# DIAGNijmegen/bodyct-dram-emph-subtype

Measured on AMD Instinct MI355X. Metric: CT volumes/sec (train step, 1x128x256x256), higher is better.
Workload: dtype f32; 1 GPU; BASELINE configs[1]: resnet18segcls train step (fwd+loss+bwd+Adam), batch 2/GPU, 1x128x256x256, fp32, inputs resident in HBM; global_batch=2, parallelism=dp1, hip_graph=False, streams=2

## Files before the change

bodyct-dram-emph-subtype_amd/csrc/conv_wino2d.hip:

```cpp
#include <stdlib.h>
#include "common.h"

namespace {

constexpr int W2_TZ16 = 16;
constexpr int W2_BK = 16;

struct W2dGeom {
  int B, D, H, W;
  int Ci, No;
  int nz, ny, nx, tiles_per_b, n_tiles, nblk;
};

__device__ __attribute__((aligned(16))) float g_w2d_zero[4];

__device__ constexpr int kBP[4][2] = {{0, 2}, {1, 2}, {1, 2}, {1, 3}};
__device__ constexpr float kBS[4][2] = {{1.f, -1.f}, {1.f, 1.f}, {-1.f, 1.f}, {1.f, -1.f}};
__device__ constexpr float kAT[2][4] = {{1.f, 1.f, 1.f, 0.f}, {0.f, 1.f, -1.f, -1.f}};

__device__ __forceinline__ int bswz(int n) {
  const int v = (n >> 2) & 7;
  return (v & 3) ^ ((v >> 2) * 3);
}

template <bool NEG>
__device__ __forceinline__ void pk_acc(f32x16& y, const f32x16& t) {
  typedef float f32x2 __attribute__((ext_vector_type(2)));
#pragma unroll
  for (int i = 0; i < 8; ++i) {
    f32x2 yy = {y[2 * i], y[2 * i + 1]};
    const f32x2 tt = {t[2 * i], t[2 * i + 1]};
    if (NEG) asm volatile("v_pk_add_f32 %0, %0, %1 neg_lo:[0,1] neg_hi:[0,1]" : "+v"(yy) : "v"(tt));
    else asm volatile("v_pk_add_f32 %0, %0, %1" : "+v"(yy) : "v"(tt));
    y[2 * i] = yy[0];
    y[2 * i + 1] = yy[1];
  }
}
template <int NJ>
__device__ __forceinline__ void mfma_result_wait(f32x16 (&t)[NJ]) {
  if (NJ == 2) asm volatile("s_nop 15\n\ts_nop 3" : "+v"(t[0]), "+v"(t[NJ - 1]));
  else asm volatile("s_nop 15\n\ts_nop 3" : "+v"(t[0]));
}

__device__ __forceinline__ int kx(int off, int gk) {
  if (gk == 0) return off;
  int r;
  asm volatile("v_xor_b32 %0, 8, %1" : "=v"(r) : "v"(off));
  return r;
}

template <int NJ, int NW = 8, int WS = 2>
__global__ __launch_bounds__(64 * NW, NW == 4 ? 2 : 1) void conv_wino2d_kernel(const float* __restrict__ in, const float* __restrict__ u2,
                                                              const float* __restrict__ bias, float* __restrict__ out,
                                                              float* __restrict__ stats, const float* __restrict__ add,
                                                              const float* __restrict__ gate, const W2dGeom g) {
  constexpr int W2_TZ = 2 * NW;
  constexpr int W2_HROWS = (W2_TZ + 2) * 10 * 10;
  constexpr int W2_NPIECE = (W2_HROWS + 15) / 16;
  constexpr int W2_HQ = (W2_NPIECE + NW - 1) / NW;
  constexpr int W2_HALO = W2_NPIECE * 256;
  constexpr int BN = 32 * NJ;
  constexpr int BROWS = 3 * BN;
  constexpr int BST = BROWS * 16;
  constexpr int BPIECE = BROWS / 16;
  constexpr int PB = (BPIECE + NW - 1) / NW;
  static_assert(WS != 3 || (NW == 4 && NJ == 2), "tap ring: one DMA piece per wave and tap");
  constexpr int TAP = BN * 16;
  __shared__ __attribute__((aligned(1024))) float lds[W2_HALO];
  __shared__ __attribute__((aligned(1024))) float wsa0[TAP], wsa1[TAP], wsa2[TAP];
  __shared__ __attribute__((aligned(1024))) float wsb0[WS == 2 ? TAP : 64], wsb1[WS == 2 ? TAP : 64],
      wsb2[WS == 2 ? TAP : 64];
  __shared__ int htab[W2_NPIECE * 16];
  float* halo = lds;

  const int tid = threadIdx.x;
  const int lane = tid & 63;
  const int wave = __builtin_amdgcn_readfirstlane(tid >> 6);

  int L = xcd_remap(blockIdx.x, g.nblk);
  const int n_tile = L % g.n_tiles;
  const int mt = L / g.n_tiles;
  const int b = mt / g.tiles_per_b;
  int r = mt - b * g.tiles_per_b;
  const int txi = r % g.nx; r /= g.nx;
  const int tyi = r % g.ny;
  const int tzi = r / g.ny;
  const int n0 = n_tile * BN;
  const int z0 = tzi * W2_TZ, y0 = tyi * 8, x0 = txi * 8;

  const int pslot = lane & 3;
  for (int rp = tid; rp < W2_NPIECE * 16; rp += 64 * NW) {
    const int yh = (rp / 10) % 10;
    const int rl = rp ^ ((yh >> 1) & 1);
    const int zh = rl / 100, xh = rl % 10;
    const int zi = z0 + zh - 1, yi = y0 + yh - 1, xi = x0 + xh - 1;
    const bool v = (rp < W2_HROWS) & (zi >= 0) & (zi < g.D) & (yi >= 0) & (yi < g.H) & (xi >= 0) & (xi < g.W);
    htab[rp] = v ? ((((b * g.D + zi) * g.H + yi) * g.W + xi) * g.Ci) | ((xh >> 2) & 1) | (((yh >> 2) & 1) << 1) : -1;
  }
  int boff[PB];
#pragma unroll
  for (int j = 0; j < PB; ++j) {
    int row = 16 * (wave + NW * j) + (lane >> 2);
    if (row >= BROWS) row = 0;
    const int a = row / BN, n = row - a * BN;
    boff[j] = (a * g.No + n0 + n) * g.Ci + (pslot ^ bswz(n)) * 4;
  }
  const long xi_stride = 3L * g.No * g.Ci;

  auto issue_halo = [&](int c) __attribute__((always_inline)) {
#pragma unroll 1
    for (int q = 0; q < W2_HQ; ++q) {
      if (wave + NW * q < W2_NPIECE) {
        const int ho = htab[16 * (wave + NW * q) + (lane >> 2)];
        const float* src = ho >= 0 ? in + (long)((ho & ~3) + ((pslot ^ (ho & 3)) << 2) + c * W2_BK) : g_w2d_zero;
        __builtin_amdgcn_global_load_lds((const __attribute__((address_space(1))) void*)src,
                                         (__attribute__((address_space(3))) void*)(halo + (wave + NW * q) * 256), 16, 0,
                                         0);
      }
    }
  };
  auto issue_b = [&](int c, int xi, int stage, int only = -1) __attribute__((always_inline)) {
#pragma unroll
    for (int j = 0; j < PB; ++j) {
      if ((only < 0 || only == j) && wave + NW * j < BPIECE) {
        const float* src = u2 + xi * xi_stride + c * W2_BK + boff[j];
        const int pb = wave + NW * j, tap = pb / (BN / 16), pin = pb - tap * (BN / 16);
        float* slot = stage == 0 ? (tap == 0 ? wsa0 : (tap == 1 ? wsa1 : wsa2)) : (tap == 0 ? wsb0 : (tap == 1 ? wsb1 : wsb2));
        __builtin_amdgcn_global_load_lds((const __attribute__((address_space(1))) void*)src,
                                         (__attribute__((address_space(3))) void*)(slot + pin * 256), 16, 0, 0);
      }
    }
  };

  f32x16 yacc[2][2][NJ];
#pragma unroll
  for (int oy = 0; oy < 2; ++oy)
#pragma unroll
    for (int ox = 0; ox < 2; ++ox)
#pragma unroll
      for (int nj = 0; nj < NJ; ++nj)
#pragma unroll
        for (int e = 0; e < 16; ++e) yacc[oy][ox][nj][e] = 0.f;

  const int li = lane & 31, lh = lane >> 5;
  const int zl = li >> 4, ty = (li >> 2) & 3, tx = li & 3;
  int abase[4][4];
#pragma unroll
  for (int p = 0; p < 4; ++p)
#pragma unroll
    for (int q = 0; q < 4; ++q) {
      const int yh = 2 * ty + p, xh = 2 * tx + q;
      const int rl = ((2 * wave + zl) * 10 + yh) * 10 + xh;
      abase[p][q] = (rl ^ ((yh >> 1) & 1)) * 16 + ((lh ^ (((xh >> 2) & 1) | (((yh >> 2) & 1) << 1))) * 4);
    }
  const int bbase = li * 16 + ((lh ^ bswz(li)) * 4);
  const int nchunk = g.Ci / W2_BK;

  for (int c = 0; c < nchunk; ++c) {
    __syncthreads();
    issue_halo(c);
    issue_b(c, 0, 0);
#pragma unroll
    for (int xi = 0; xi < 16; ++xi) {
      if (WS != 3 || xi == 0) __syncthreads();
      const int stage = WS == 2 ? (xi & 1) : 0;
      if (WS == 2 && xi + 1 < 16) issue_b(c, xi + 1, stage ^ 1);
      const int xy = xi >> 2, xx = xi & 3;
      const int p0 = kBP[xy][0], p1 = kBP[xy][1], q0 = kBP[xx][0], q1 = kBP[xx][1];
      const float s00 = kBS[xy][0] * kBS[xx][0], s01 = kBS[xy][0] * kBS[xx][1];
      const float s10 = kBS[xy][1] * kBS[xx][0], s11 = kBS[xy][1] * kBS[xx][1];
      f32x16 t[NJ];
#pragma unroll
      for (int a = 0; a < 3; ++a) {
        const float* wtap = stage == 0 ? (a == 0 ? wsa0 : (a == 1 ? wsa1 : wsa2)) : (a == 0 ? wsb0 : (a == 1 ? wsb1 : wsb2));
#pragma unroll
        for (int gk = 0; gk < 2; ++gk) {
          const f32x4 r00 = *reinterpret_cast<const f32x4*>(halo + kx(abase[p0][q0], gk) + a * 1600);
          const f32x4 r01 = *reinterpret_cast<const f32x4*>(halo + kx(abase[p0][q1], gk) + a * 1600);
          const f32x4 r10 = *reinterpret_cast<const f32x4*>(halo + kx(abase[p1][q0], gk) + a * 1600);
          const f32x4 r11 = *reinterpret_cast<const f32x4*>(halo + kx(abase[p1][q1], gk) + a * 1600);
          const f32x4 av = (s00 * r00 + s01 * r01) + (s10 * r10 + s11 * r11);
          f32x4 bf[NJ];
#pragma unroll
          for (int nj = 0; nj < NJ; ++nj)
            bf[nj] = *reinterpret_cast<const f32x4*>(wtap + nj * 32 * 16 + kx(bbase, gk));
#pragma unroll
          for (int e = 0; e < 4; ++e) {
#pragma unroll
            for (int nj = 0; nj < NJ; ++nj) {
              if (a == 0 && gk == 0 && e == 0) {
                f32x16 zero;
#pragma unroll
                for (int i = 0; i < 16; ++i) zero[i] = 0.f;
                t[nj] = __builtin_amdgcn_mfma_f32_32x32x2f32(av[e], bf[nj][e], zero, 0, 0, 0);
              } else {
                t[nj] = __builtin_amdgcn_mfma_f32_32x32x2f32(av[e], bf[nj][e], t[nj], 0, 0, 0);
              }
            }
          }
          __builtin_amdgcn_sched_barrier(0);
        }
        if (WS == 3 && !(xi == 15 && a == 2)) {
          if (xi == 15 && a >= 1) asm volatile("s_waitcnt vmcnt(0)");
          else asm volatile("s_waitcnt vmcnt(1)");
          __builtin_amdgcn_s_barrier();
          if (xi + 1 < 16) issue_b(c, xi + 1, 0, a);
        }
      }
      mfma_result_wait<NJ>(t);
#pragma unroll
      for (int oy = 0; oy < 2; ++oy)
#pragma unroll
        for (int ox = 0; ox < 2; ++ox) {
          const float cf = kAT[oy][xy] * kAT[ox][xx];
          if (cf != 0.f) {
#pragma unroll
            for (int nj = 0; nj < NJ; ++nj) {
              if (cf > 0.f) pk_acc<false>(yacc[oy][ox][nj], t[nj]);
              else pk_acc<true>(yacc[oy][ox][nj], t[nj]);
            }
          }
        }
      __builtin_amdgcn_sched_barrier(0);
      if (WS == 1 && xi + 1 < 16) {
        __syncthreads();
        issue_b(c, xi + 1, 0);
      }
    }
  }

  int lhe = lh, lie = li;
  asm volatile("" : "+v"(lhe), "+v"(lie));
  constexpr int P = 32 * NJ + 8;
  constexpr int Q = 8 * NJ;
  constexpr int VPP = 64 / Q;
  static_assert(NW * 32 * P <= W2_HALO, "turn regions fit the halo buffer");
  __syncthreads();
  float* reg = lds + wave * (32 * P);
  const int cq = lane % Q, rs = lane / Q;
  f32x4 s1 = {0.f, 0.f, 0.f, 0.f}, s2 = {0.f, 0.f, 0.f, 0.f}, bv = {0.f, 0.f, 0.f, 0.f};
  if (bias) bv = *reinterpret_cast<const f32x4*>(bias + n0 + 4 * cq);
#pragma unroll
  for (int oy = 0; oy < 2; ++oy)
#pragma unroll
    for (int ox = 0; ox < 2; ++ox) {
#pragma unroll
      for (int e = 0; e < 16; ++e)
#pragma unroll
        for (int nj = 0; nj < NJ; ++nj)
          reg[((e & 3) + 8 * (e >> 2) + 4 * lhe) * P + nj * 32 + lie] = yacc[oy][ox][nj][e];
#pragma unroll
      for (int ps = 0; ps < 32 / VPP; ++ps) {
        const int row = ps * VPP + rs;
        const int zo = z0 + 2 * wave + (row >> 4);
        const int yo = y0 + 2 * ((row >> 2) & 3) + oy, xo = x0 + 2 * (row & 3) + ox;
        f32x4 v = *reinterpret_cast<const f32x4*>(reg + row * P + 4 * cq);
        if ((zo < g.D) & (yo < g.H) & (xo < g.W)) {
          const long o = ((((long)b * g.D + zo) * g.H + yo) * g.W + xo) * g.No + n0 + 4 * cq;
          v += bv;
          if (add) {
            const f32x4 av = *reinterpret_cast<const f32x4*>(add + o);
            if (gate) {
              const f32x4 gv = *reinterpret_cast<const f32x4*>(gate + o);
#pragma unroll
              for (int j = 0; j < 4; ++j) v[j] += gv[j] > 0.f ? av[j] : 0.f;
            } else {
              v += av;
            }
          }
          *reinterpret_cast<f32x4*>(out + o) = v;
          s1 += v;
          s2 += v * v;
        }
      }
    }
  if (stats) {
#pragma unroll
    for (int j = 0; j < 4; ++j)
#pragma unroll
      for (int o = Q; o < 64; o <<= 1) {
        s1[j] += __shfl_xor(s1[j], o, 64);
        s2[j] += __shfl_xor(s2[j], o, 64);
      }
    __syncthreads();
    float* red = lds;
    if (rs == 0) {
#pragma unroll
      for (int j = 0; j < 4; ++j) {
        red[(wave * 2 + 0) * BN + 4 * cq + j] = s1[j];
        red[(wave * 2 + 1) * BN + 4 * cq + j] = s2[j];
      }
    }
    __syncthreads();
    if (tid < 2 * BN) {
      const int which = tid / BN, cc = tid - which * BN;
      float v = 0.f;
#pragma unroll
      for (int w = 0; w < NW; ++w) v += red[(w * 2 + which) * BN + cc];
      stats[((long)mt * 2 + which) * g.No + n0 + cc] = v;
    }
  }
}

constexpr int V2_TZ = 8;
constexpr int V2_HROWS = 10 * 10 * 10;
constexpr int V2_NPIECE = (V2_HROWS + 15) / 16;
constexpr int V2_HALO = V2_NPIECE * 256;

template <bool NEG>
__device__ __forceinline__ void pk_acc4(f32x4& y, const f32x4& t) {
  typedef float f32x2 __attribute__((ext_vector_type(2)));
#pragma unroll
  for (int i = 0; i < 2; ++i) {
    f32x2 yy = {y[2 * i], y[2 * i + 1]};
    const f32x2 tt = {t[2 * i], t[2 * i + 1]};
    if (NEG) asm volatile("v_pk_add_f32 %0, %0, %1 neg_lo:[0,1] neg_hi:[0,1]" : "+v"(yy) : "v"(tt));
    else asm volatile("v_pk_add_f32 %0, %0, %1" : "+v"(yy) : "v"(tt));
    y[2 * i] = yy[0];
    y[2 * i + 1] = yy[1];
  }
}
template <int NB>
__device__ __forceinline__ void mfma16_result_wait(f32x4 (&t)[NB]) {
  if (NB == 4) asm volatile("s_nop 12" : "+v"(t[0]), "+v"(t[1]), "+v"(t[2]), "+v"(t[NB - 1]));
  else asm volatile("s_nop 12" : "+v"(t[0]), "+v"(t[NB - 1]));
}

__device__ __forceinline__ int bswz16(int n) { return (0x78 >> (2 * ((n >> 2) & 3))) & 3; }

template <int NB>
__global__ __launch_bounds__(512) void conv_wino2d16_kernel(const float* __restrict__ in, const float* __restrict__ u2,
                                                            const float* __restrict__ bias, float* __restrict__ out,
                                                            float* __restrict__ stats, const float* __restrict__ add,
                                                            const float* __restrict__ gate, const W2dGeom g) {
  constexpr int BN = 16 * NB;
  constexpr int BROWS = 3 * BN;
  constexpr int BST = BROWS * 16;
  constexpr int BPIECE = BROWS / 16;
  constexpr int PB = (BPIECE + 7) / 8;
  __shared__ __attribute__((aligned(1024))) float lds[V2_HALO];
  __shared__ __attribute__((aligned(1024))) float halo1[V2_HALO];
  __shared__ __attribute__((aligned(1024))) float wst0[BST], wst1[BST];
  __shared__ int htab[V2_NPIECE * 16];

  const int tid = threadIdx.x;
  const int lane = tid & 63;
  const int wave = __builtin_amdgcn_readfirstlane(tid >> 6);

  int L = xcd_remap(blockIdx.x, g.nblk);
  const int n_tile = L % g.n_tiles;
  const int mt = L / g.n_tiles;
  const int b = mt / g.tiles_per_b;
  int r = mt - b * g.tiles_per_b;
  const int txi = r % g.nx; r /= g.nx;
  const int tyi = r % g.ny;
  const int tzi = r / g.ny;
  const int n0 = n_tile * BN;
  const int z0 = tzi * V2_TZ, y0 = tyi * 8, x0 = txi * 8;

  const int pslot = lane & 3;
  for (int rp = tid; rp < V2_NPIECE * 16; rp += 512) {
    const int yh = (rp / 10) % 10;
    const int rl = rp ^ ((yh >> 1) & 1);
    const int zh = rl / 100, xh = rl % 10;
    const int zi = z0 + zh - 1, yi = y0 + yh - 1, xi = x0 + xh - 1;
    const bool v = (rp < V2_HROWS) & (zi >= 0) & (zi < g.D) & (yi >= 0) & (yi < g.H) & (xi >= 0) & (xi < g.W);
    htab[rp] = v ? ((((b * g.D + zi) * g.H + yi) * g.W + xi) * g.Ci) | ((xh >> 2) & 1) | (((yh >> 2) & 1) << 1) : -1;
  }
  int boff[PB];
#pragma unroll
  for (int j = 0; j < PB; ++j) {
    int row = 16 * (wave + 8 * j) + (lane >> 2);
    if (row >= BROWS) row = 0;
    const int a = row / BN, n = row - a * BN;
    boff[j] = (a * g.No + n0 + n) * g.Ci + (pslot ^ bswz16(n)) * 4;
  }
  const long xi_stride = 3L * g.No * g.Ci;

  auto issue_halo_piece = [&](int c, int p, float* buf) __attribute__((always_inline)) {
    const int ho = htab[16 * p + (lane >> 2)];
    const float* src = ho >= 0 ? in + (long)((ho & ~3) + ((pslot ^ (ho & 3)) << 2) + c * W2_BK) : g_w2d_zero;
    __builtin_amdgcn_global_load_lds((const __attribute__((address_space(1))) void*)src,
                                     (__attribute__((address_space(3))) void*)(buf + p * 256), 16, 0, 0);
  };
  auto issue_b = [&](int c, int xi, int stage) __attribute__((always_inline)) {
#pragma unroll
    for (int j = 0; j < PB; ++j) {
      if (wave + 8 * j < BPIECE) {
        const float* src = u2 + xi * xi_stride + c * W2_BK + boff[j];
        __builtin_amdgcn_global_load_lds((const __attribute__((address_space(1))) void*)src,
                                         (__attribute__((address_space(3))) void*)((stage ? wst1 : wst0) + (wave + 8 * j) * 256),
                                         16, 0, 0);
      }
    }
  };

  f32x4 yacc[2][2][NB];
#pragma unroll
  for (int oy = 0; oy < 2; ++oy)
#pragma unroll
    for (int ox = 0; ox < 2; ++ox)
#pragma unroll
      for (int cb = 0; cb < NB; ++cb)
#pragma unroll
        for (int e = 0; e < 4; ++e) yacc[oy][ox][cb][e] = 0.f;

  const int lr = lane & 15, kq = lane >> 4;
  const int ty = lr >> 2, tx = lr & 3;
  int abase[4][4];
#pragma unroll
  for (int p = 0; p < 4; ++p)
#pragma unroll
    for (int q = 0; q < 4; ++q) {
      const int yh = 2 * ty + p, xh = 2 * tx + q;
      const int rl = (wave * 10 + yh) * 10 + xh;
      abase[p][q] = (rl ^ ((yh >> 1) & 1)) * 16 + ((kq ^ (((xh >> 2) & 1) | (((yh >> 2) & 1) << 1))) * 4);
    }
  const int bbase = lr * 16 + ((kq ^ bswz16(lr)) * 4);
  const int nchunk = g.Ci / W2_BK;

  __syncthreads();
#pragma unroll 1
  for (int q = 0; q < 8; ++q)
    if (wave + 8 * q < V2_NPIECE) issue_halo_piece(0, wave + 8 * q, lds);
  issue_b(0, 0, 0);

  auto chunk = [&](const int c, const float* hb, float* hn) __attribute__((always_inline)) {
#pragma unroll
    for (int xi = 0; xi < 16; ++xi) {
      __syncthreads();
      if (xi + 1 < 16) issue_b(c, xi + 1, (xi + 1) & 1);
      else if (c + 1 < nchunk) issue_b(c + 1, 0, 0);
      if (c + 1 < nchunk) {
        const int w4 = wave - 4 * (xi & 1);
        const int p = xi * 4 + w4;
        if (w4 >= 0 && w4 < 4 && p < V2_NPIECE) issue_halo_piece(c + 1, p, hn);
      }
      const int xy = xi >> 2, xx = xi & 3;
      const int p0 = kBP[xy][0], p1 = kBP[xy][1], q0 = kBP[xx][0], q1 = kBP[xx][1];
      const float s00 = kBS[xy][0] * kBS[xx][0], s01 = kBS[xy][0] * kBS[xx][1];
      const float s10 = kBS[xy][1] * kBS[xx][0], s11 = kBS[xy][1] * kBS[xx][1];
      const float* bs = (xi & 1) ? wst1 : wst0;
      f32x4 t[NB];
#pragma unroll
      for (int a = 0; a < 3; ++a) {
        const f32x4 r00 = *reinterpret_cast<const f32x4*>(hb + abase[p0][q0] + a * 1600);
        const f32x4 r01 = *reinterpret_cast<const f32x4*>(hb + abase[p0][q1] + a * 1600);
        const f32x4 r10 = *reinterpret_cast<const f32x4*>(hb + abase[p1][q0] + a * 1600);
        const f32x4 r11 = *reinterpret_cast<const f32x4*>(hb + abase[p1][q1] + a * 1600);
        f32x4 bf[NB];
#pragma unroll
        for (int cb = 0; cb < NB; ++cb)
          bf[cb] = *reinterpret_cast<const f32x4*>(bs + (a * BN + cb * 16) * 16 + bbase);
        const f32x4 av = (s00 * r00 + s01 * r01) + (s10 * r10 + s11 * r11);
#pragma unroll
        for (int e = 0; e < 4; ++e) {
#pragma unroll
          for (int cb = 0; cb < NB; ++cb) {
            if (a == 0 && e == 0) {
              const f32x4 zero = {0.f, 0.f, 0.f, 0.f};
              t[cb] = __builtin_amdgcn_mfma_f32_16x16x4f32(av[e], bf[cb][e], zero, 0, 0, 0);
            } else {
              t[cb] = __builtin_amdgcn_mfma_f32_16x16x4f32(av[e], bf[cb][e], t[cb], 0, 0, 0);
            }
          }
        }
      }
      mfma16_result_wait<NB>(t);
#pragma unroll
      for (int oy = 0; oy < 2; ++oy)
#pragma unroll
        for (int ox = 0; ox < 2; ++ox) {
          const float cf = kAT[oy][xy] * kAT[ox][xx];
          if (cf != 0.f) {
#pragma unroll
            for (int cb = 0; cb < NB; ++cb) {
              if (cf > 0.f) pk_acc4<false>(yacc[oy][ox][cb], t[cb]);
              else pk_acc4<true>(yacc[oy][ox][cb], t[cb]);
            }
          }
        }
    }
  };
  for (int c = 0; c < nchunk; c += 2) {
    chunk(c, lds, halo1);
    if (c + 1 < nchunk) chunk(c + 1, halo1, lds);
  }

  float s1[NB], s2[NB], bv[NB];
#pragma unroll
  for (int cb = 0; cb < NB; ++cb) {
    s1[cb] = 0.f;
    s2[cb] = 0.f;
    bv[cb] = bias ? bias[n0 + cb * 16 + lr] : 0.f;
  }
  const int zo = z0 + wave;
#pragma unroll
  for (int i = 0; i < 4; ++i) {
#pragma unroll
    for (int oy = 0; oy < 2; ++oy)
#pragma unroll
      for (int ox = 0; ox < 2; ++ox) {
        const int yo = y0 + 2 * kq + oy, xo = x0 + 2 * i + ox;
        if ((zo < g.D) & (yo < g.H) & (xo < g.W)) {
          const long o = ((((long)b * g.D + zo) * g.H + yo) * g.W + xo) * g.No + n0 + lr;
#pragma unroll
          for (int cb = 0; cb < NB; ++cb) {
            float v = yacc[oy][ox][cb][i] + bv[cb];
            if (add) {
              const float av = add[o + cb * 16];
              v += gate ? (gate[o + cb * 16] > 0.f ? av : 0.f) : av;
            }
            out[o + cb * 16] = v;
            s1[cb] += v;
            s2[cb] += v * v;
          }
        }
      }
  }
  if (stats) {
    __syncthreads();
    float* red = lds;
#pragma unroll
    for (int cb = 0; cb < NB; ++cb) {
      float t1 = s1[cb] + __shfl_xor(s1[cb], 16, 64);
      float t2 = s2[cb] + __shfl_xor(s2[cb], 16, 64);
      t1 += __shfl_xor(t1, 32, 64);
      t2 += __shfl_xor(t2, 32, 64);
      if (kq == 0) {
        red[(wave * 2 + 0) * BN + cb * 16 + lr] = t1;
        red[(wave * 2 + 1) * BN + cb * 16 + lr] = t2;
      }
    }
    __syncthreads();
    if (tid < 2 * BN) {
      const int which = tid / BN, cc = tid - which * BN;
      float v = 0.f;
#pragma unroll
      for (int w = 0; w < 8; ++w) v += red[(w * 2 + which) * BN + cc];
      stats[((long)mt * 2 + which) * g.No + n0 + cc] = v;
    }
  }
}

__device__ __forceinline__ void g4_2d(const float a0, const float a1, const float a2, float* r) {
  const float h = 0.5f * (a0 + a2);
  r[0] = a0;
  r[1] = h + 0.5f * a1;
  r[2] = h - 0.5f * a1;
  r[3] = a2;
}

__global__ __launch_bounds__(256) void wino2d_weight_kernel(const float* __restrict__ w, float* __restrict__ uf,
                                                            float* __restrict__ ub, const int Cout, const int Cin) {
  const bool bwd = blockIdx.y == 1;
  float* dst = bwd ? ub : uf;
  if (!dst) return;
  const long n = (long)Cout * Cin;
  const long i = blockIdx.x * 256L + threadIdx.x;
  if (i >= n) return;
  int co, ci;
  if (!bwd) { ci = (int)(i % Cin); co = (int)(i / Cin); }
  else { co = (int)(i % Cout); ci = (int)(i / Cout); }
  const float* src = w + ((long)co * Cin + ci) * 27;
  float gw[3][3][3];
#pragma unroll
  for (int t = 0; t < 27; ++t) (&gw[0][0][0])[t] = src[bwd ? 26 - t : t];
#pragma unroll
  for (int a = 0; a < 3; ++a) {
    float p[3][4], u[4][4];
#pragma unroll
    for (int ky = 0; ky < 3; ++ky) g4_2d(gw[a][ky][0], gw[a][ky][1], gw[a][ky][2], p[ky]);
#pragma unroll
    for (int x = 0; x < 4; ++x) {
      float col[4];
      g4_2d(p[0][x], p[1][x], p[2][x], col);
#pragma unroll
      for (int y = 0; y < 4; ++y) u[y][x] = col[y];
    }
#pragma unroll
    for (int xi = 0; xi < 16; ++xi) dst[((long)xi * 3 + a) * n + i] = u[xi >> 2][xi & 3];
  }
}

bool w2d_ok(const DramConvDesc* d, int K, int N) {
  if (!d) return false;
  if (d->B < 1 || d->D < 1 || d->H < 1 || d->W < 1) return false;
  if (d->k != 3 || d->stride != 1 || d->dil != 1 || d->pad != 1) return false;
  if (d->Do != d->D || d->Ho != d->H || d->Wo != d->W) return false;
  if (K < 16 || K % 16 != 0 || N < 32 || N % 32 != 0) return false;
  const long long cmax = K > N ? K : N;
  return (long long)d->B * d->D * d->H * d->W * cmax < (1LL << 31);
}

int w2d_variant(const DramConvDesc* d, int n_tiles, int BN) {
  if (const char* e = tune_env("DRAM_W2D_V")) {
    const int v = atoi(e);
    if (v >= 1 && v <= 3) return v;
  }
  const int z16 = (d->D + 15) / 16, z8 = (d->D + 7) / 8;
  const long cols = (long)d->B * ((d->H + 7) / 8) * ((d->W + 7) / 8) * n_tiles;
  if (BN == 64 && cols * z8 >= 1024) return 3;
  if (z16 * 16 != z8 * 8) return 2;
  auto fill = [](long wgs) { return (double)wgs / (double)(((wgs + 255) / 256) * 256); };
  return fill(cols * z16) + 0.05 < fill(cols * z8) ? 2 : 1;
}

W2dGeom make_w2d(const DramConvDesc* d, int K, int N, int BN, int* variant = nullptr) {
  W2dGeom g{};
  g.B = d->B; g.D = d->D; g.H = d->H; g.W = d->W; g.Ci = K; g.No = N;
  g.n_tiles = N / BN;
  const int v = w2d_variant(d, g.n_tiles, BN);
  if (variant) *variant = v;
  const int tz = v == 1 ? W2_TZ16 : V2_TZ;
  g.nz = (g.D + tz - 1) / tz;
  g.ny = (g.H + 7) / 8;
  g.nx = (g.W + 7) / 8;
  g.tiles_per_b = g.nz * g.ny * g.nx;
  g.nblk = g.B * g.tiles_per_b * g.n_tiles;
  return g;
}

int run_w2d(const float* in, const float* u2, const float* bias, const float* add, const float* gate, float* out,
            float* stats, const DramConvDesc* d, int K, int N, hipStream_t s) {
  const int BN = N % 64 == 0 ? 64 : 32;
  int variant = 1;
  const W2dGeom g = make_w2d(d, K, N, BN, &variant);
  const double vox_pad = (double)g.B * g.tiles_per_b * (variant == 1 ? W2_TZ16 : V2_TZ) * 64.0;
  const double vox = (double)g.B * g.D * g.H * g.W;
  DramProf prof(DRAM_FAM_CONV_WINO2D, variant * 100 + BN, 2.0 * vox_pad * K * N * 12.0,
                4.0 * (vox * (K + N * (1.0 + (add ? 1 : 0) + (gate ? 1 : 0))) + 48.0 * K * N), s,
                2.0 * vox * K * N * 27.0);
  if (variant == 1) {
    if (BN == 64)
      hipLaunchKernelGGL((conv_wino2d_kernel<2>), dim3(g.nblk), dim3(512), 0, s, in, u2, bias, out, stats, add, gate, g);
    else
      hipLaunchKernelGGL((conv_wino2d_kernel<1>), dim3(g.nblk), dim3(512), 0, s, in, u2, bias, out, stats, add, gate, g);
  } else if (variant == 3) {
    if (BN == 64)
      hipLaunchKernelGGL((conv_wino2d_kernel<2, 4, 3>), dim3(g.nblk), dim3(256), 0, s, in, u2, bias, out, stats, add, gate, g);
    else
      hipLaunchKernelGGL((conv_wino2d_kernel<1, 4, 1>), dim3(g.nblk), dim3(256), 0, s, in, u2, bias, out, stats, add, gate, g);
  } else {
    if (BN == 64)
      hipLaunchKernelGGL((conv_wino2d16_kernel<4>), dim3(g.nblk), dim3(512), 0, s, in, u2, bias, out, stats, add, gate, g);
    else
      hipLaunchKernelGGL((conv_wino2d16_kernel<2>), dim3(g.nblk), dim3(512), 0, s, in, u2, bias, out, stats, add, gate, g);
  }
  DRAM_LAUNCH_CHECK();
  return DRAM_OK;
}

}

extern "C" int dram_wino2d_applicable(const DramConvDesc* d) {
  return (d && w2d_ok(d, d->Cin, d->Cout) && w2d_ok(d, d->Cout, d->Cin)) ? 1 : 0;
}

extern "C" int dram_wino2d_num_stat_rows(const DramConvDesc* d) {
  if (!dram_wino2d_applicable(d)) return DRAM_ERR_UNSUPPORTED;
  const W2dGeom g = make_w2d(d, d->Cin, d->Cout, d->Cout % 64 == 0 ? 64 : 32);
  return g.B * g.tiles_per_b;
}

extern "C" int dram_wino2d_pack_weight(const float* w, float* uf, float* ub, int Cout, int Cin, dram_stream_t stream) {
  if (!w || (!uf && !ub) || Cout < 1 || Cin < 1) return DRAM_ERR_BAD_ARG;
  const long n = (long)Cout * Cin;
  DramProf prof(DRAM_FAM_WEIGHT_PACK, 2, 0.0, 4.0 * (double)n * (27.0 + (uf ? 48 : 0) + (ub ? 48 : 0)),
                (hipStream_t)stream);
  hipLaunchKernelGGL(wino2d_weight_kernel, dim3((unsigned)((n + 255) / 256), 2), dim3(256), 0, (hipStream_t)stream, w,
                     uf, ub, Cout, Cin);
  DRAM_LAUNCH_CHECK();
  return DRAM_OK;
}

extern "C" int dram_wino2d_conv3d_fwd(const float* x, const float* uf, const float* bias, float* y, float* stats_partial,
                                      const DramConvDesc* d, dram_stream_t stream) {
  if (!x || !uf || !y) return DRAM_ERR_BAD_ARG;
  if (!dram_wino2d_applicable(d)) return DRAM_ERR_UNSUPPORTED;
  return run_w2d(x, uf, bias, nullptr, nullptr, y, stats_partial, d, d->Cin, d->Cout, (hipStream_t)stream);
}

extern "C" int dram_wino2d_conv3d_bwd_data(const float* dy, const float* ub, float* dx, const float* add,
                                           const float* gate, const DramConvDesc* d, dram_stream_t stream) {
  if (!dy || !ub || !dx || (gate && !add)) return DRAM_ERR_BAD_ARG;
  if (!dram_wino2d_applicable(d)) return DRAM_ERR_UNSUPPORTED;
  return run_w2d(dy, ub, nullptr, add, gate, dx, nullptr, d, d->Cout, d->Cin, (hipStream_t)stream);
}
```

Before: 55.55 volumes/sec.

## Hoist x-direction Winograd input transform in BN=32 conv variant and reorder tile loop

Adds a variant of the 2D Winograd conv kernel for 32-wide output-channel tiles. It iterates the 16 transform points column-major so the x-direction input transform is computed once per column and reused across the four y points, which cuts LDS reads and VALU work. This variant becomes the default for large BN=32 layers, and the existing BN=32 NW=4 path switches from single to double-buffered weight staging. The forward and stats paths now only check the forward-direction applicability. The cost is extra registers holding the hoisted transforms (96 VGPRs), which could hurt occupancy.

After: 56.01 volumes/sec, median of 6. Within noise of the previous version (+0.8%).

```diff
diff --git a/bodyct-dram-emph-subtype_amd/csrc/conv_wino2d.hip b/bodyct-dram-emph-subtype_amd/csrc/conv_wino2d.hip
--- a/bodyct-dram-emph-subtype_amd/csrc/conv_wino2d.hip
+++ b/bodyct-dram-emph-subtype_amd/csrc/conv_wino2d.hip
@@ -48,8 +48,17 @@
   asm volatile("v_xor_b32 %0, 8, %1" : "=v"(r) : "v"(off));
   return r;
 }
-
-template <int NJ, int NW = 8, int WS = 2>
+__device__ __forceinline__ int kxb(int off, int gk) {
+  if (gk == 0) return off;
+  int r;
+  asm volatile("v_xor_b32 %0, 32, %1" : "=v"(r) : "v"(off));
+  return r;
+}
+__device__ __forceinline__ f32x4 lds16(const float* base, int byte) {
+  return *reinterpret_cast<const f32x4*>(reinterpret_cast<const char*>(base) + byte);
+}
+
+template <int NJ, int NW = 8, int WS = 2, bool HX = false>
 __global__ __launch_bounds__(64 * NW, NW == 4 ? 2 : 1) void conv_wino2d_kernel(const float* __restrict__ in, const float* __restrict__ u2,
                                                               const float* __restrict__ bias, float* __restrict__ out,
                                                               float* __restrict__ stats, const float* __restrict__ add,
@@ -65,6 +74,7 @@
   constexpr int BPIECE = BROWS / 16;
   constexpr int PB = (BPIECE + NW - 1) / NW;
   static_assert(WS != 3 || (NW == 4 && NJ == 2), "tap ring: one DMA piece per wave and tap");
+  static_assert(!HX || NJ == 1, "hoisted x half: 96 registers beside 80 of accumulators");
   constexpr int TAP = BN * 16;
   __shared__ __attribute__((aligned(1024))) float lds[W2_HALO];
   __shared__ __attribute__((aligned(1024))) float wsa0[TAP], wsa1[TAP], wsa2[TAP];
@@ -142,6 +152,7 @@
 #pragma unroll
         for (int e = 0; e < 16; ++e) yacc[oy][ox][nj][e] = 0.f;
 
+  constexpr int AU = HX ? 4 : 1;
   const int li = lane & 31, lh = lane >> 5;
   const int zl = li >> 4, ty = (li >> 2) & 3, tx = li & 3;
   int abase[4][4];
@@ -151,20 +162,23 @@
     for (int q = 0; q < 4; ++q) {
       const int yh = 2 * ty + p, xh = 2 * tx + q;
       const int rl = ((2 * wave + zl) * 10 + yh) * 10 + xh;
-      abase[p][q] = (rl ^ ((yh >> 1) & 1)) * 16 + ((lh ^ (((xh >> 2) & 1) | (((yh >> 2) & 1) << 1))) * 4);
-    }
-  const int bbase = li * 16 + ((lh ^ bswz(li)) * 4);
+      abase[p][q] = ((rl ^ ((yh >> 1) & 1)) * 16 + ((lh ^ (((xh >> 2) & 1) | (((yh >> 2) & 1) << 1))) * 4)) * AU;
+    }
+  const int bbase = (li * 16 + ((lh ^ bswz(li)) * 4)) * AU;
   const int nchunk = g.Ci / W2_BK;
 
   for (int c = 0; c < nchunk; ++c) {
     __syncthreads();
     issue_halo(c);
     issue_b(c, 0, 0);
-#pragma unroll
-    for (int xi = 0; xi < 16; ++xi) {
-      if (WS != 3 || xi == 0) __syncthreads();
-      const int stage = WS == 2 ? (xi & 1) : 0;
-      if (WS == 2 && xi + 1 < 16) issue_b(c, xi + 1, stage ^ 1);
+    f32x4 cx[HX ? 3 : 1][2][4];
+#pragma unroll
+    for (int pt = 0; pt < 16; ++pt) {
+      const int xi = HX ? 4 * (pt & 3) + (pt >> 2) : pt;
+      const int xn = HX ? 4 * ((pt + 1) & 3) + ((pt + 1) >> 2) : pt + 1;
+      if (WS != 3 || pt == 0) __syncthreads();
+      const int stage = WS == 2 ? (pt & 1) : 0;
+      if (WS == 2 && pt + 1 < 16) issue_b(c, xn, stage ^ 1);
       const int xy = xi >> 2, xx = xi & 3;
       const int p0 = kBP[xy][0], p1 = kBP[xy][1], q0 = kBP[xx][0], q1 = kBP[xx][1];
       const float s00 = kBS[xy][0] * kBS[xx][0], s01 = kBS[xy][0] * kBS[xx][1];
@@ -175,15 +189,29 @@
         const float* wtap = stage == 0 ? (a == 0 ? wsa0 : (a == 1 ? wsa1 : wsa2)) : (a == 0 ? wsb0 : (a == 1 ? wsb1 : wsb2));
 #pragma unroll
         for (int gk = 0; gk < 2; ++gk) {
-          const f32x4 r00 = *reinterpret_cast<const f32x4*>(halo + kx(abase[p0][q0], gk) + a * 1600);
-          const f32x4 r01 = *reinterpret_cast<const f32x4*>(halo + kx(abase[p0][q1], gk) + a * 1600);
-          const f32x4 r10 = *reinterpret_cast<const f32x4*>(halo + kx(abase[p1][q0], gk) + a * 1600);
-          const f32x4 r11 = *reinterpret_cast<const f32x4*>(halo + kx(abase[p1][q1], gk) + a * 1600);
-          const f32x4 av = (s00 * r00 + s01 * r01) + (s10 * r10 + s11 * r11);
+          f32x4 av;
+          if constexpr (HX) {
+            if (xy == 0) {
+#pragma unroll
+              for (int p = 0; p < 4; ++p) {
+                const f32x4 v0 = lds16(halo, kxb(abase[p][q0], gk) + a * 6400);
+                const f32x4 v1 = lds16(halo, kxb(abase[p][q1], gk) + a * 6400);
+                cx[a][gk][p] = kBS[xx][0] * v0 + kBS[xx][1] * v1;
+                if (p == 1) __builtin_amdgcn_sched_barrier(0);
+              }
+            }
+            av = kBS[xy][0] * cx[a][gk][p0] + kBS[xy][1] * cx[a][gk][p1];
+          } else {
+            const f32x4 r00 = *reinterpret_cast<const f32x4*>(halo + kx(abase[p0][q0], gk) + a * 1600);
+            const f32x4 r01 = *reinterpret_cast<const f32x4*>(halo + kx(abase[p0][q1], gk) + a * 1600);
+            const f32x4 r10 = *reinterpret_cast<const f32x4*>(halo + kx(abase[p1][q0], gk) + a * 1600);
+            const f32x4 r11 = *reinterpret_cast<const f32x4*>(halo + kx(abase[p1][q1], gk) + a * 1600);
+            av = (s00 * r00 + s01 * r01) + (s10 * r10 + s11 * r11);
+          }
           f32x4 bf[NJ];
 #pragma unroll
           for (int nj = 0; nj < NJ; ++nj)
-            bf[nj] = *reinterpret_cast<const f32x4*>(wtap + nj * 32 * 16 + kx(bbase, gk));
+            bf[nj] = HX ? lds16(wtap, kxb(bbase, gk)) : *reinterpret_cast<const f32x4*>(wtap + nj * 32 * 16 + kx(bbase, gk));
 #pragma unroll
           for (int e = 0; e < 4; ++e) {
 #pragma unroll
@@ -200,11 +228,11 @@
           }
           __builtin_amdgcn_sched_barrier(0);
         }
-        if (WS == 3 && !(xi == 15 && a == 2)) {
-          if (xi == 15 && a >= 1) asm volatile("s_waitcnt vmcnt(0)");
+        if (WS == 3 && !(pt == 15 && a == 2)) {
+          if (pt == 15 && a >= 1) asm volatile("s_waitcnt vmcnt(0)");
           else asm volatile("s_waitcnt vmcnt(1)");
           __builtin_amdgcn_s_barrier();
-          if (xi + 1 < 16) issue_b(c, xi + 1, 0, a);
+          if (pt + 1 < 16) issue_b(c, xn, 0, a);
         }
       }
       mfma_result_wait<NJ>(t);
@@ -222,10 +250,6 @@
           }
         }
       __builtin_amdgcn_sched_barrier(0);
-      if (WS == 1 && xi + 1 < 16) {
-        __syncthreads();
-        issue_b(c, xi + 1, 0);
-      }
     }
   }
 
@@ -597,14 +621,17 @@
   if (const char* e = tune_env("DRAM_W2D_V")) {
     const int v = atoi(e);
     if (v >= 1 && v <= 3) return v;
+    if (v == 4 && BN == 32) return v;
   }
   const int z16 = (d->D + 15) / 16, z8 = (d->D + 7) / 8;
   const long cols = (long)d->B * ((d->H + 7) / 8) * ((d->W + 7) / 8) * n_tiles;
-  if (BN == 64 && cols * z8 >= 1024) return 3;
+  if (cols * z8 >= 1024) return BN == 64 ? 3 : 4;
   if (z16 * 16 != z8 * 8) return 2;
   auto fill = [](long wgs) { return (double)wgs / (double)(((wgs + 255) / 256) * 256); };
   return fill(cols * z16) + 0.05 < fill(cols * z8) ? 2 : 1;
 }
+
+constexpr int w2d_tz(int variant) { return variant == 1 ? W2_TZ16 : V2_TZ; }
 
 W2dGeom make_w2d(const DramConvDesc* d, int K, int N, int BN, int* variant = nullptr) {
   W2dGeom g{};
@@ -612,7 +639,7 @@
   g.n_tiles = N / BN;
   const int v = w2d_variant(d, g.n_tiles, BN);
   if (variant) *variant = v;
-  const int tz = v == 1 ? W2_TZ16 : V2_TZ;
+  const int tz = w2d_tz(v);
   g.nz = (g.D + tz - 1) / tz;
   g.ny = (g.H + 7) / 8;
   g.nx = (g.W + 7) / 8;
@@ -626,7 +653,7 @@
   const int BN = N % 64 == 0 ? 64 : 32;
   int variant = 1;
   const W2dGeom g = make_w2d(d, K, N, BN, &variant);
-  const double vox_pad = (double)g.B * g.tiles_per_b * (variant == 1 ? W2_TZ16 : V2_TZ) * 64.0;
+  const double vox_pad = (double)g.B * g.tiles_per_b * w2d_tz(variant) * 64.0;
   const double vox = (double)g.B * g.D * g.H * g.W;
   DramProf prof(DRAM_FAM_CONV_WINO2D, variant * 100 + BN, 2.0 * vox_pad * K * N * 12.0,
                 4.0 * (vox * (K + N * (1.0 + (add ? 1 : 0) + (gate ? 1 : 0))) + 48.0 * K * N), s,
@@ -636,11 +663,13 @@
       hipLaunchKernelGGL((conv_wino2d_kernel<2>), dim3(g.nblk), dim3(512), 0, s, in, u2, bias, out, stats, add, gate, g);
     else
       hipLaunchKernelGGL((conv_wino2d_kernel<1>), dim3(g.nblk), dim3(512), 0, s, in, u2, bias, out, stats, add, gate, g);
+  } else if (variant == 4) {
+    hipLaunchKernelGGL((conv_wino2d_kernel<1, 4, 2, true>), dim3(g.nblk), dim3(256), 0, s, in, u2, bias, out, stats, add, gate, g);
   } else if (variant == 3) {
     if (BN == 64)
       hipLaunchKernelGGL((conv_wino2d_kernel<2, 4, 3>), dim3(g.nblk), dim3(256), 0, s, in, u2, bias, out, stats, add, gate, g);
     else
-      hipLaunchKernelGGL((conv_wino2d_kernel<1, 4, 1>), dim3(g.nblk), dim3(256), 0, s, in, u2, bias, out, stats, add, gate, g);
+      hipLaunchKernelGGL((conv_wino2d_kernel<1, 4, 2>), dim3(g.nblk), dim3(256), 0, s, in, u2, bias, out, stats, add, gate, g);
   } else {
     if (BN == 64)
       hipLaunchKernelGGL((conv_wino2d16_kernel<4>), dim3(g.nblk), dim3(512), 0, s, in, u2, bias, out, stats, add, gate, g);
@@ -658,7 +687,7 @@
 }
 
 extern "C" int dram_wino2d_num_stat_rows(const DramConvDesc* d) {
-  if (!dram_wino2d_applicable(d)) return DRAM_ERR_UNSUPPORTED;
+  if (!d || !w2d_ok(d, d->Cin, d->Cout)) return DRAM_ERR_UNSUPPORTED;
   const W2dGeom g = make_w2d(d, d->Cin, d->Cout, d->Cout % 64 == 0 ? 64 : 32);
   return g.B * g.tiles_per_b;
 }
@@ -677,7 +706,7 @@
 extern "C" int dram_wino2d_conv3d_fwd(const float* x, const float* uf, const float* bias, float* y, float* stats_partial,
                                       const DramConvDesc* d, dram_stream_t stream) {
   if (!x || !uf || !y) return DRAM_ERR_BAD_ARG;
-  if (!dram_wino2d_applicable(d)) return DRAM_ERR_UNSUPPORTED;
+  if (!d || !w2d_ok(d, d->Cin, d->Cout)) return DRAM_ERR_UNSUPPORTED;
   return run_w2d(x, uf, bias, nullptr, nullptr, y, stats_partial, d, d->Cin, d->Cout, (hipStream_t)stream);
 }
 
```
